# lanl-ansi/Katana.jl

Hardware: AMD Instinct MI355X
Metric: ECP iterations/sec + wall-clock to f_tol=1e-6, 1e5-var synthetic convex NLP (higher is better)
Workload: dtype f64; 1 GPU; cfg3: n=100000 variables, m_lin=50000 linear rows (8 nnz), m_nl=10000 explog rows (k=32 nnz), seed 0, planted non-degenerate vertex optimum, f_tol=1e-6; parallelism=1 GPU

## Files before the change

### katana.jl_amd/csrc/engine.hpp

```cpp
#pragma once
#include <hip/hip_runtime.h>

#include <algorithm>
#include <chrono>
#include <cstdlib>
#include <cmath>
#include <limits>
#include <map>
#include <string>
#include <vector>

#include <rccl/rccl.h>

#include "common.hpp"
#include "types.hpp"
#include "prims.hpp"

namespace ktn {

static const double kInf = std::numeric_limits<double>::infinity();

static inline int pick_group(double avg_len) {
    int g = 4;
    while (g < 64 && 2 * g <= avg_len) g <<= 1;
    return g;
}

struct LpResult {
    int status = KTN_STATUS_NONE;
    int64_t iters = 0;
    double pobj = 0.0, dobj = 0.0, row_viol = 0.0, gap = 0.0;
    double dres_rel = 0.0;
    bool exact = false;
    bool stag_exit = false;
};

struct DevParams {
    bool no_pinned_check = false, debug_load = false, no_csc_merge = false, tiled_general_build = false, debug_blocks = false,
         no_tiled_check = false, no_setup_reuse = false, debug_lp = false, no_packed = false, force_collective = false;
    int sweep_rows = 0;
    int blk_cfg = -1;
    int sweep_blocked = -1;
    int sweep_batched = -1;
    int tape_classed = -1;
    int tiled_wg = 2;
    int ecp_power = 20;
    int grp_rows = 0, grp_cols = 0;
    int tiled = -1;
    double smax_reuse = 0.0;
    int power_passes = 0;
    int omega_robust = 1;
    int packed_trips = 0;
    int first_chunk = 31;
    int stag_chunk = 0;
    int near_chunk = -1;
    int stag_checks = 2;
    double flat_factor = 0.4;
    int omega_art = 1;
    double omega_art_k = 256.0;
    double omega_art_clamp = 0.0, omega_clamp = 0.0, omega_clamp_down = 0.0;
    double ipc_timeout_s = 20.0;
    static bool flag(const char* k) { return std::getenv(k) != nullptr; }
    static int geti(const char* k, int d) { const char* v = std::getenv(k); return v ? std::atoi(v) : d; }
    static double getd(const char* k, double d) { const char* v = std::getenv(k); return v ? std::atof(v) : d; }
    void from_env() {
        no_pinned_check = flag("KTN_NO_PINNED_CHECK"); debug_load = flag("KTN_DEBUG_LOAD"); no_csc_merge = flag("KTN_NO_CSC_MERGE");
        tiled_general_build = flag("KTN_TILED_GENERAL_BUILD"); debug_blocks = flag("KTN_DEBUG_BLOCKS"); no_tiled_check = flag("KTN_NO_TILED_CHECK");
        no_setup_reuse = flag("KTN_NO_SETUP_REUSE"); debug_lp = flag("KTN_DEBUG_LP"); no_packed = flag("KTN_NO_PACKED");
        force_collective = flag("KTN_FORCE_COLLECTIVE");
        sweep_rows = geti("KTN_SWEEP_ROWS", sweep_rows); blk_cfg = geti("KTN_BLK_CFG", blk_cfg); sweep_blocked = geti("KTN_SWEEP_BLOCKED", sweep_blocked);
        sweep_batched = geti("KTN_SWEEP_BATCHED", sweep_batched); tape_classed = geti("KTN_TAPE_CLASSED", tape_classed);
        tiled_wg = geti("KTN_TILED_WG", tiled_wg); ecp_power = geti("KTN_ECP_POWER", ecp_power);
        grp_rows = geti("KTN_GRP_ROWS", grp_rows); grp_cols = geti("KTN_GRP_COLS", grp_cols); tiled = geti("KTN_TILED", tiled);
        smax_reuse = getd("KTN_SMAX_REUSE", smax_reuse); power_passes = geti("KTN_POWER_PASSES", power_passes);
        omega_robust = geti("KTN_OMEGA_ROBUST", omega_robust); packed_trips = geti("KTN_PACKED_TRIPS", packed_trips);
        first_chunk = geti("KTN_FIRST_CHUNK", first_chunk); stag_chunk = geti("KTN_STAG_CHUNK", stag_chunk); near_chunk = geti("KTN_NEAR_CHUNK", near_chunk);
        stag_checks = geti("KTN_STAG_CHECKS", stag_checks); flat_factor = getd("KTN_FLAT_FACTOR", flat_factor);
        omega_art = geti("KTN_OMEGA_ART", omega_art); omega_art_k = getd("KTN_OMEGA_ART_K", omega_art_k);
        omega_art_clamp = getd("KTN_OMEGA_ART_CLAMP", omega_art_clamp); omega_clamp = getd("KTN_OMEGA_CLAMP", omega_clamp);
        omega_clamp_down = getd("KTN_OMEGA_CLAMP_DOWN", omega_clamp_down); ipc_timeout_s = getd("KTN_IPC_TIMEOUT_S", ipc_timeout_s);
    }
};

struct Engine {
    ktn_params prm;
    DevParams dev;
    std::string err;
    hipStream_t stream = nullptr;
    int device = 0;

    bool loaded = false;
    int64_t n0 = 0, m0 = 0;
    int64_t n_lp = 0;
    int64_t m_ext = 0;
    int64_t nnz_ext = 0;
    int sense = KTN_MIN;
    bool obj_linear = true;
    bool has_inf_bound = false;
    std::vector<int64_t> h_rowptr;
    std::vector<int32_t> h_col;
    std::vector<uint8_t> h_rowkind;
    std::vector<double> h_lb, h_ub;
    std::vector<int32_t> h_nlrows;
    int64_t m_nl = 0, n_tape_nl = 0;
    int64_t m_nl_global = 0;
    int grp_sweep = 32;
    int sweep_rows_per_group = 1;
    bool pre_multirow = false;

    DBuf<int64_t> d_rowptr, d_nodeptr;
    DBuf<int32_t> d_col, d_nodeop, d_nodea, d_nodeb;
    DBuf<uint8_t> d_rowkind, d_padzero;
    DBuf<uint64_t> d_dkeys, d_dsorted;
    ktn_eval_rows_cb cb_rows = nullptr;
    ktn_eval_obj_cb cb_obj = nullptr;
    void* cb_user = nullptr;
    int64_t n_host = 0, n_host_nl = 0;
    bool host_constr_rows = false, host_obj = false;
    std::vector<double> h_xh, h_gh, h_jh;
    DBuf<double> d_gh, d_jh;
    DBuf<int32_t> d_hostrows;
    void host_eval(const double* d_x);
    DBuf<int32_t> d_colk;
    DBuf<double2> d_pp;
    bool blk_on = false;
    int blk_nb = 0, blk_cfg = 0, blk_cols = kBlkCols, blk_wg_per_cu = 2, num_cus = 256;
    DBuf<int32_t> d_bcolk;
    DBuf<double2> d_bpp;
    DBuf<int64_t> d_bseg;
    DBuf<int4> d_bkind;
    DBuf<SepSlot> d_slots;
    DBuf<SepPartial> d_part;
    DBuf<double> d_rconst, d_lb, d_ub, d_nodec, d_nodeval, d_nodeadj;
// ... 31 lines not shown
    bool lp_dirty = true;
    uint64_t lp_version = 1, scaled_version = 0, smax_version = 0;
    bool scaled_identity = false;
    ktn_exchange_cb exch_cb = nullptr;
    void* exch_user = nullptr;
    int64_t exch_lo = 0;
    bool exchanging() const { return exch_cb != nullptr; }
    bool sharded_rows = false;
    bool glists = false;
    int64_t nl_total = 0;
    int64_t last_sweep_cuts = 0;
    DBuf<int64_t> d_glast, d_nlid;
    void append_link(int64_t nrows, const int64_t* nl_id_host);
    void append_link_dev(int64_t nrows);
    int64_t* list_heads() { return glists ? d_glast.p : d_lastcut.p; }
    int64_t list_count() const { return glists ? nl_total : m_nl; }
    bool lists_ok() const { return !sharded_rows || glists; }
    DBuf<int64_t> c_ptr, c_cnt;
    DBuf<int32_t> c_row;
    DBuf<double> c_val, c_sval, r_sval;
    DBuf<uint32_t> c_perm, c_perm2;
    DBuf<int32_t> c_row2;
    DBuf<int64_t> c_ptr2, c_off;
    int64_t csc_M = -1, csc_NNZ = 0;
    uint64_t lp_epoch = 1, csc_epoch = 0;
    void csc_merge_appended();
    bool w_shift = false;
    int64_t M_lin = 0;
    DBuf<double> wval, wlo, whi, wc, epi_ref, epi_scal;
    DBuf<unsigned long long> epi_newest;
    const double* Wval() const { return w_shift ? wval.p : lp_val.p; }
    const double* Wlo() const { return w_shift ? wlo.p : lp_lo.p; }
    const double* Whi() const { return w_shift ? whi.p : lp_hi.p; }
    const double* Wc() const { return w_shift ? wc.p : lp_c.p; }
    bool want_shift(int mode) const { return prm.epi_shift != 0 && !obj_linear && mode == 0 && !row_sharded() && n_blocks == 0; }
    void build_working();
    void ensure_matrix(bool shift);
    void epi_dot(const double* x);
    DBuf<uint64_t> k_in, k_out;
    DBuf<uint32_t> p_in, p_out;
    DBuf<char> d_sorttmp;
    DBuf<double> dr_r, dc_r;
    DBuf<ColRec> d_crec;
    DBuf<RowRec> d_rrec;
    DBuf<int2> d_cbl;
    bool packed_on = false;
    int packed_trips = 1;
    DBuf<double> dr2, dc2;
    DBuf<double> dr, dc, statr, statc, ch, lh, uh, loh, hih, xh, yh, x0h, y0h, xth, yth, xbar, pv, pw, box;
    DBuf<double> partials, chk_part, chkout, power_v, power_v0;
    int64_t power_v0_n = -1;
    double* h_chk = nullptr;
    double* h_chk_dev = nullptr;
    int64_t lp_iter_budget = 0, dense_credit = 0, dense_run = 0;
    DBuf<int32_t> ds_W, ds_valid;
    DBuf<double> ds_dense, ds_out;
    DBuf<double> md_Binv, md_hW, md_x, md_lam, md_u, md_d, md_r, md_pv, md_c, md_aug, md_prow, md_fcol;
    int64_t md_since_refactor = 0;
    int64_t mid_backoff = 0, mid_backoff_len = 0;
    DBuf<int32_t> md_W, md_pi, md_lost;
    DBuf<MidState> md_st;
    bool md_valid = false;
    int64_t mid_credit = 0, mid_run = 0;
    DBuf<int32_t> d_longrows;
    DBuf<int32_t> d_longcols;
    int64_t n_longc = 0;
    int64_t col_gain_max = 0;
    int64_t col_len_max = -1, col_scan_rows = 0;
    int64_t col_removed_rows = 0;
    void find_long_cols();
    void spmv_cols(const SpMat& AT, const double* v, double* out, hipEvent_t e0 = nullptr, hipEvent_t e1 = nullptr);
    static constexpr int kMaxChunk = 512;
    int64_t n_long = 0;
    static constexpr int64_t kLongRow = 2048;
    int64_t max_row_len = (int64_t)1 << 62;
    double omega = 1.0;
    bool have_omega = false;
    int grp_rows = 8, grp_cols = 8;
    struct TiledBuf {
        DBuf<int64_t> segstart, segtot;
        DBuf<uint16_t> bptr, cur, idx;
        DBuf<int32_t> pcnt;
        DBuf<double> val;
        int nb_in = 0;
        int64_t tiles = 0, grid = 0, pieces = 1;
        TiledMat view() const { return TiledMat{segstart.p, bptr.p, idx.p, val.p, nb_in}; }
    } tA, tAT;
    DBuf<double> tpart;
    bool tiled_on = false, tiled_built = false;
    void launch_tiled(const TiledBuf& T, int64_t n_out, int64_t n_in, const double* in, hipEvent_t e0);
    bool build_tiled(TiledBuf& T, int64_t n_out, int64_t n_in, const int64_t* ptr, const int32_t* idx, const double* val, int64_t skip_longer);
    int64_t n_blocks = 0, blocks_built_rows = -1;
    size_t lds_set_lp = 0, lds_set_ecp = 0;
    std::vector<int64_t> h_blkcol;
    DBuf<int64_t> d_blkcol;
    DBuf<int32_t> d_blkrowptr, d_blkrows, d_rowloc, d_crowl;
    DBuf<double> d_blkomega, d_blkres;
    int blk_nmax = 0, blk_mmax = 0;
    void build_blocks();
    bool optimize_blocks_device(int cap_mul);
    DBuf<EcpArena> d_ar;
    DBuf<int64_t> d_blklin, d_blknl;
    DBuf<int32_t> e_rptr, e_cptr, e_last, e_prev;
    DBuf<uint16_t> e_rcol, e_crow;
    DBuf<double> e_xbest, e_ax, e_rval, e_rsval, e_lo, e_hi, e_y, e_dr, e_loh, e_hih, e_cval, e_csval, e_dc, e_ch, e_lh, e_uh, e_res;
    bool lp_solve_blocks(double tol_p, double tol_g, double eta, LpResult* R, int64_t max_it);
// ... 12 lines not shown
    int polish_count = 0;
    double polish_phi = 1e-3;
    double cert_target = 0.0;
    double cert_gap = 0.0;
    DBuf<double> d_cert;
    double objective_certificate(int64_t id_offset = 0, bool raw = false);
    double certificate_all_ranks();
    bool sweep_all(const double* d_x, double f_cut, bool lp_ok, int lp_stat, int64_t* nviol, double* maxviol, double* extra0, double* extra1);
    double certificate_blocks(double* gap_tol);
    DBuf<double> d_certblk;
    double best_viol = kInf, best_obj = 0.0;
    DBuf<double> d_xbest;
    int64_t log_cuts_lastprnt = 0, log_max_viol = 0, purged_total = 0;
    bool logging() const { return prm.log_level > 0 && dist.rank == 0; }
    void print_header() const {
        std::printf("%-10s %-15s %-15s %-20s %-20s %-15s\n", "Iteration", "Total cuts", "Cuts added", "Max constr. viol.",
                    "Avg constr. viol.", "Current cuts");
    }
    void print_stats(int64_t iter_lastprnt) const {
        const double avg = (double)log_cuts_lastprnt / ((double)iter_lastprnt * (double)m_nl);
        std::printf("%-10lld %-15lld %-15lld %-20lld %-20.2f %-15lld\n", (long long)iter, (long long)numcuts,
                    (long long)log_cuts_lastprnt, (long long)log_max_viol, avg, (long long)(numcuts - purged_total));
        std::fflush(stdout);
    }
    std::chrono::steady_clock::time_point t_start;
    std::vector<std::vector<double>> lp_sols;
    std::map<std::string, double> stats;
    std::vector<hipEvent_t> ev_pool;
    struct EvRec { int kind; size_t a, b; double bytes; };
    std::vector<EvRec> ev_recs;
    size_t ev_used = 0;

    explicit Engine(const ktn_params& p) : prm(p) {
        dev.from_env();
        if (prm.cut_algo != KTN_CUT_KELLEY && prm.cut_algo != KTN_CUT_SUPPORTING)
            throw Error(KTN_E_INVALID, "cut_algo must be KTN_CUT_KELLEY (0) or KTN_CUT_SUPPORTING (1)");
        int ndev = 0;
        if (hipGetDeviceCount(&ndev) != hipSuccess || ndev <= 0)
            throw Error(KTN_E_NODEVICE, "no HIP device visible: the Katana HIP engine has no CPU path");
        if (prm.device >= 0) {
            KTN_HIP(hipSetDevice(prm.device));
            device = prm.device;
        } else {
            KTN_HIP(hipGetDevice(&device));
        }
        {
            int cus = 0;
            if (hipDeviceGetAttribute(&cus, hipDeviceAttributeMultiprocessorCount, device) == hipSuccess && cus > 0) num_cus = cus;
        }
        KTN_HIP(hipStreamCreateWithFlags(&stream, hipStreamNonBlocking));
        partials.resize((size_t)kRedBlocks * kChkQ * 2, stream);
        chkout.resize(kChkQ * 2 + 16, stream);
        if (!dev.no_pinned_check &&
            hipHostMalloc((void**)&h_chk, sizeof(double) * (2 * kChkQ + 16), hipHostMallocMapped) == hipSuccess) {
            if (hipHostGetDevicePointer((void**)&h_chk_dev, h_chk, 0) != hipSuccess) { (void)hipHostFree(h_chk); h_chk = nullptr; h_chk_dev = nullptr; }
        } else {
            h_chk = nullptr;
            (void)hipGetLastError();
        }
        d_scal.resize(8, stream);
        d_anynf.resize(4, stream);
    }
    ~Engine() {
        delete child;
        if (dist.comm) (void)ncclCommDestroy(dist.comm);
        ipc_release();
        for (auto e : ev_pool) (void)hipEventDestroy(e);
        if (stream) (void)hipStreamDestroy(stream);
        if (h_chk) (void)hipHostFree(h_chk);
    }

    void sync() { KTN_HIP(hipStreamSynchronize(stream)); }
    bool chk_pinned() const { return h_chk_dev != nullptr && !row_sharded(); }
    double* chk_target() { return chk_pinned() ? h_chk_dev : chkout.p; }
    void check_launch() { KTN_HIP(hipGetLastError()); }

    struct DistCtx {
        int rank = 0, world = 1;
        bool force = false;
        ncclComm_t comm = nullptr;
        ktn_allreduce_cb cb = nullptr;
        void* user = nullptr;
        std::vector<double> hbuf;
        struct Ipc {
            bool on = false;
            int64_t cap = 0;
            double* data = nullptr;
            unsigned long long* flags = nullptr;
            void* opened[2 * kIpcMaxRanks] = {};
            IpcPeers P = {};
            unsigned long long epoch = 0;
            long long timeout_ticks = 0;
            int* h_err = nullptr;
            int* h_err_dev = nullptr;
        } ipc;
    } dist;
    int64_t ipc_off() const { return (int64_t)(dist.ipc.epoch & 1ull) * dist.ipc.cap; }
    double* ipc_slot() const { return dist.ipc.data + ipc_off(); }
    void ipc_check() {
        if (dist.ipc.on && dist.ipc.h_err && *dist.ipc.h_err != 0) {
            const int code = *dist.ipc.h_err;
            if (code > 100)
                throw Error(KTN_E_HIP, "peer-buffer transport: rank " + std::to_string(code - 101) + " gave up (told rank " + std::to_string(dist.rank) + ")");
            throw Error(KTN_E_HIP, "peer-buffer transport: rank " + std::to_string(dist.rank) + " timed out waiting for rank " + std::to_string(code - 1));
        }
    }
    int64_t ipc_barrier();
    void ipc_release();
    void probe_fill(int64_t n, double* v, double value);
    DBuf<double> d_red;
    bool row_sharded() const { return dist.world > 1 || dist.force; }
    void allreduce(double* d, size_t n, int op);
    void allreduce_host(double* v, int k, int op);

    size_t ev_get() {
        if (ev_used == ev_pool.size()) {
            hipEvent_t e;
            KTN_HIP(hipEventCreate(&e));
            ev_pool.push_back(e);
        }
// ... 48 lines not shown
    DBuf<double2> d_sbpp;
    DBuf<int64_t> d_sbseg;

    std::vector<int8_t> h_esh_side;
    DBuf<int8_t> d_esh_sig;
    DBuf<double> d_xint, d_lam;
    DBuf<int32_t> d_tape_nlslots;
    DBuf<unsigned long long> d_esh_cnt;
    std::vector<double> h_xint;
    bool xint_given = false, esh_ready = false;
    int xint_found = 0;
    int64_t esh_n_part = 0;
    struct EshAux {
        int64_t n = 0, m = 0;
        std::vector<double> lv, uv, lc, uc, rconst, p0, p1, targ, op0, op1;
        std::vector<int64_t> rowptr, tptr;
        std::vector<int32_t> col, top, ocol;
        std::vector<uint8_t> kind, lin, akind, okind;
        bool has_tape = false;
    } aux;
    Engine* child = nullptr;
    void esh_build_aux(const double* l_var, const double* u_var, const double* l_constr, const double* u_constr, const ktn_nlp_desc* d);
    void esh_prepare();
    void esh_find_interior();
    bool esh_on = false;
    int64_t esh_last_rows = 0;
    void esh_search(const double* d_x, double f_tol);
    void esh_emit(const double* d_x, int64_t V);
    DBuf<int32_t> d_esh_one;
    DBuf<int64_t> d_esh_slot;
    bool esh_gencut_row(int64_t i, double* coefs, double* constant);
    void esh_last_lambdas(double* out);

    void rebuild_csc();
    void purge_cuts();
    void reserve_lp(int64_t rows, int64_t nnz);
    void find_long_rows();
    bool recession_ray_dense(bool* unbounded);
    void launch_y(const SpMat& A, double sigma, double w, double rho, hipEvent_t e0, hipEvent_t e1);
    void launch_x(const SpMat& AT, double tau, double w, double rho, bool update, hipEvent_t e0, hipEvent_t e1);
    bool launch_check(const SpMat& A, const SpMat& AT, double tau, double sigma, double w_next = -1.0, double rho = 1.0);
    DBuf<double> xnext, ynext;
    int chk_nrow = 0, chk_ncol = 0;
    void compute_scaling(bool identity);
    LpResult lp_solve(double tol_p, double tol_g, int mode, bool identity_scaling = false);
    LpResult lp_solve_core(double tol_p, double tol_g, int mode, bool identity_scaling);
    bool lp_solve_dense(LpResult* R);
    bool lp_solve_mid(LpResult* R);
    void pdhg_raw(const double* x0, const double* y0, double eta, double omega_, int64_t iters, double* x_out,
                  double* y_out);
    void lp_pick_groups();
    void lp_choose_tiled(bool same_matrix);
    void lp_set_anchors(bool want_packed);
    void lp_read_check(double* q);
    void lp_restart();
    void lp_advance(bool spec, int64_t k, double rho);
    struct LpScriptIO {
        const double *x, *y, *x0, *y0;
        double eta, omega;
        int64_t k;
        int32_t flags;
        const int32_t* ops;
        int64_t nops;
        double *x_out, *y_out, *x0_out, *y0_out, *xt_out, *yt_out, *q_out, *xnext_out, *ynext_out;
        int32_t* spec_out;
        double *dr_out, *dc_out;
    };
    void lp_script(const LpScriptIO& io);
    void lp_scaling(double* dr_out, double* dc_out, double* drr_out, double* dcr_out);

    bool recession_ray();
    void boundroutine();
    void begin();
    void step(int32_t* done);
    void polish_step(int32_t* done);
    void end();
};

}
```

### katana.jl_amd/csrc/lp.hip

```cpp
#include "engine.hpp"
#include "launch.hpp"
#include "kernels.hpp"
#include "dense_lp.hpp"
#include "mid_lp.hpp"
#include "batch_lp.hpp"

namespace ktn {

double Engine::dev_dot(int64_t n, const double* a, const double* b) {
    hipLaunchKernelGGL(k_dot_partial, dim3(kRedBlocks), dim3(kBlock), 0, stream, n, a, b, partials.p);
    hipLaunchKernelGGL(k_sum_final, dim3(1), dim3(kRedBlocks), 0, stream, partials.p, kRedBlocks, chkout.p + 2 * kChkQ);
    double v = 0.0;
    KTN_HIP(hipMemcpyAsync(&v, chkout.p + 2 * kChkQ, sizeof(double), hipMemcpyDeviceToHost, stream));
    sync();
    return v;
}

double Engine::dev_finite_sq(int64_t n, const double* a) {
    hipLaunchKernelGGL(k_finite_sq_partial, dim3(kRedBlocks), dim3(kBlock), 0, stream, n, a, partials.p);
    hipLaunchKernelGGL(k_sum_final, dim3(1), dim3(kRedBlocks), 0, stream, partials.p, kRedBlocks, chkout.p + 2 * kChkQ);
    double v = 0.0;
    KTN_HIP(hipMemcpyAsync(&v, chkout.p + 2 * kChkQ, sizeof(double), hipMemcpyDeviceToHost, stream));
    sync();
    return v;
// ... 601 lines not shown
        md_valid = false;
        ok = true;
    }
    stats["lp_time_s"] += std::chrono::duration<double>(std::chrono::steady_clock::now() - t0).count();
    return ok;
}

void Engine::lp_pick_groups() {
    const int64_t n = n_lp, m = M;
    const double avg_r = m ? (double)NNZ / (double)m : 1.0, avg_c = n ? (double)NNZ / (double)n : 1.0;
    grp_rows = pick_group(avg_r);
    grp_cols = pick_group(avg_c);
    if (dev.grp_rows > 0) grp_rows = dev.grp_rows;
    if (dev.grp_cols > 0) grp_cols = dev.grp_cols;
}

void Engine::lp_choose_tiled(bool same_matrix) {
    {
        const bool tenv = dev.tiled >= 0;
        const int64_t units_t = ceil_div(M, (int64_t)kTileOut) * ceil_div(n_lp, (int64_t)kTileIn);
        const int64_t units_tt = ceil_div(n_lp, (int64_t)kTileOut) * ceil_div(M, (int64_t)kTileIn);
        tiled_on = prm.lp_tiled_nnz > 0 && NNZ >= prm.lp_tiled_nnz && n_lp >= 2 * kTileIn && M >= 2 * kTileIn &&
                   NNZ >= 4096 * std::max(units_t, units_tt);
        if (tenv) tiled_on = dev.tiled != 0 && M > 0 && NNZ > 0;
        if (same_matrix) tiled_on = tiled_built;
        else if (tiled_on) {
            auto tt = std::chrono::steady_clock::now();
            tiled_on = build_tiled(tA, M, n_lp, lp_rowptr.p, lp_col.p, r_sval.p, kLongRow) &&
                       build_tiled(tAT, n_lp, M, c_ptr.p, c_row.p, c_sval.p, (int64_t)1 << 62);
            tpart.resize((size_t)std::max<int64_t>(tA.pieces * M, tAT.pieces * n_lp), stream);
            stats["lp_tiled_builds"] += 1.0;
            stats["lp_tiled_build_time_s"] += std::chrono::duration<double>(std::chrono::steady_clock::now() - tt).count();
            if (!tiled_on) stats["lp_tiled_overflows"] += 1.0;
        }
        tiled_built = tiled_on;
    }
}

void Engine::lp_set_anchors(bool want_packed) {
    const int64_t n = n_lp, m = M;
    const size_t mm = (size_t)std::max<int64_t>(m, 1);
    packed_on = want_packed && !tiled_on && !row_sharded() && NNZ < ((int64_t)1 << 31) && !dev.no_packed;
    if (dev.packed_trips > 0) packed_trips = dev.packed_trips;
    if (packed_on) {
        d_crec.resize((size_t)n, stream); d_cbl.resize((size_t)n, stream); d_rrec.resize(mm, stream);
        LAUNCH_1(k_pack_both, std::max(n, m), stream, n, c_ptr.p, ch.p, lh.p, uh.p, xh.p, x0h.p, d_crec.p, d_cbl.p,
                 m, lp_rowptr.p, loh.p, hih.p, yh.p, y0h.p, d_rrec.p);
    } else {
        KTN_HIP(hipMemcpyAsync(x0h.p, xh.p, n * sizeof(double), hipMemcpyDeviceToDevice, stream));
        if (m > 0) KTN_HIP(hipMemcpyAsync(y0h.p, yh.p, m * sizeof(double), hipMemcpyDeviceToDevice, stream));
    }
}

void Engine::lp_read_check(double* q) {
    if (chk_pinned()) {
        sync();
        std::memcpy(q, h_chk, 2 * kChkQ * sizeof(double));
    } else {
        KTN_HIP(hipMemcpyAsync(q, chkout.p, 2 * kChkQ * sizeof(double), hipMemcpyDeviceToHost, stream));
        sync();
        ipc_check();
    }
}

void Engine::lp_restart() {
    const int64_t n = n_lp, m = M;
    LAUNCH_1(k_restart_set, std::max(n, m), stream, n, m, xth.p, xh.p, x0h.p, yth.p, yh.p, y0h.p, packed_on ? d_crec.p : (ColRec*)nullptr,
             packed_on ? d_rrec.p : (RowRec*)nullptr);
}

void Engine::lp_advance(bool spec, int64_t k, double rho) {
    const int64_t n = n_lp, m = M;
    if (spec) {
        xh.swap(xnext); yh.swap(ynext);
    } else {
        const double w = (double)(k + 1) / (double)(k + 2);
        LAUNCH_1(k_halpern2, std::max(n, m), stream, n, m, xh.p, xth.p, x0h.p, yh.p, yth.p, y0h.p, w, rho);
    }
}

LpResult Engine::lp_solve_core(double tol_p, double tol_g, int mode, bool identity_scaling) {
    auto t0 = std::chrono::steady_clock::now();
    LpResult R;
    auto lap = [&](const char* key, std::chrono::steady_clock::time_point& tp) {
        if (!prm.profile) return;
        sync();
        const auto now = std::chrono::steady_clock::now();
        stats[key] += std::chrono::duration<double>(now - tp).count();
        tp = now;
    };
    auto tp = t0;
    ensure_matrix(want_shift(mode));
    lap("lp_csc_time_s", tp);
    const bool no_reuse = dev.no_setup_reuse;
    const bool same_matrix = !no_reuse && !row_sharded() && scaled_version == lp_version && scaled_identity == identity_scaling;
    find_long_rows();
    if (!same_matrix) compute_scaling(identity_scaling);
    else stats["lp_setup_reuses"] += 1.0;
    lap("lp_scaling_time_s", tp);
    const int64_t n = n_lp, m = M;
    const size_t mm = (size_t)std::max<int64_t>(m, 1);
    ch.resize(n, stream); lh.resize(n, stream); uh.resize(n, stream); xh.resize(n, stream);
    x0h.resize(n, stream); xth.resize(n, stream); xbar.resize(n, stream); pv.resize(n, stream);
    loh.resize(mm, stream); hih.resize(mm, stream); yh.resize(mm, stream); y0h.resize(mm, stream);
    yth.resize(mm, stream); pw.resize(mm, stream);
    const double sgn = (sense == KTN_MAX) ? -1.0 : 1.0;
    LAUNCH_1(k_prep_both, std::max(n, m), stream,
             PrepCols{n, Wc(), lp_l.p, lp_u.p, dc.p, lp_x.p, (mode == 1 ? box.p : (const double*)nullptr), sgn, mode, ch.p, lh.p, uh.p, xh.p},
             PrepRows{m, Wlo(), Whi(), dr.p, lp_y.p, mode, loh.p, hih.p, yh.p});
    if (w_shift) {
        epi_dot(lp_x.p);
        hipLaunchKernelGGL(k_epi_var, dim3(1), dim3(1), 0, stream, xh.p, (int32_t)n0, epi_scal.p, (const double*)dc.p, -1, have_omega ? 0 : 1, sgn, epi_newest.p);
    }
    check_launch();
    lp_pick_groups();
    SpMat A{lp_rowptr.p, lp_col.p, r_sval.p};
    SpMat AT{c_ptr.p, c_row.p, c_sval.p};
    lp_choose_tiled(same_matrix);
    scaled_version = lp_version; scaled_identity = identity_scaling;

    double smax = 0.0;
    bool have_power = false;
    const double smax_reuse = dev.smax_reuse;
    const bool reuse_smax = mode == 0 && smax_reuse > 0.0 && smax_rows > 0 && m >= smax_rows && !row_sharded() &&
                            (double)(m - smax_rows) <= smax_reuse * (double)smax_rows && smax_prev > 0.0;
    if (same_matrix && smax_version == lp_version && smax_prev > 0.0) smax = smax_prev;
    else if (reuse_smax) { smax = smax_prev; stats["lp_smax_reused"] += 1.0; }
    else if ((m > 0 && NNZ > 0) || row_sharded()) {
        double* nrm = (chk_pinned() ? h_chk_dev : chkout.p) + 2 * kChkQ + 1;
        auto dot_dev = [&](const double* a, double* out) {
            hipLaunchKernelGGL(k_dot_partial, dim3(kRedBlocks), dim3(kBlock), 0, stream, n, a, a, partials.p);
            hipLaunchKernelGGL(k_sum_final, dim3(1), dim3(kRedBlocks), 0, stream, partials.p, kRedBlocks, out);
        };
        auto normalize_into = [&](const double* a, double* out) {
            hipLaunchKernelGGL(k_dot_partial, dim3(kRedBlocks), dim3(kBlock), 0, stream, n, a, a, partials.p);
            hipLaunchKernelGGL(k_normalize_sum, dim3(ceil_div(n, (int64_t)kRedBlocks)), dim3(kRedBlocks), 0, stream, n, a, partials.p, out);
        };
        if (power_v0_n != n) {
            power_v.resize(n, stream); power_v0.resize(n, stream);
            LAUNCH_1(k_hash_fill, n, stream, n, power_v.p);
            normalize_into(power_v.p, power_v0.p);
            power_v0_n = n;
        }
        const int passes_env = dev.power_passes;
        const int iters = passes_env > 0 ? passes_env : 8;
        for (int it = 0; it < iters; ++it) {
            const double* vin = (it == 0) ? power_v0.p : pv.p;
            if (n_long > 0) {
                LAUNCH_G(grp_rows, k_spmv_skip, m, stream, m, A, vin, pw.p, kLongRow);
// ... 44 lines not shown
        const double nv2 = hs[1];
        smax = (nv2 > 0.0) ? std::sqrt(std::sqrt(nv2)) : 0.0;
        if (mode == 0) { smax_prev = smax; smax_rows = m; smax_version = lp_version; }
    }
    lap("lp_power_time_s", tp);
    double fro2 = (NNZ > 0) ? hs[2] : 0.0;
    allreduce_host(&fro2, 1, 0);
    const double fro = std::sqrt(fro2);
    if (!(smax > 0.0)) smax = fro;
    const double eta_safe = 0.998 / std::max(identity_scaling ? fro : std::min(1.0, fro), 1e-12);
    double eta = std::max(0.998 / std::max(smax, 1e-12), eta_safe);
    int stall = 0, grow = 0, flat_rows = 0, consolidations = 0, infeas_hits = 0;
    double pobj_h[3] = {1e300, -1e300, 1e300}, pviol_h[3] = {1e300, -1e300, 1e300};
    double r_last_check = 0.0;
    stats["lp_setup_time_s"] += std::chrono::duration<double>(std::chrono::steady_clock::now() - t0).count();
    const double nc2 = hs[3];
    const double nc2_tol = w_shift ? hs[6] : nc2;
    double nb2 = (m > 0) ? hs[4] + hs[5] : 0.0;
    allreduce_host(&nb2, 1, 0);
    double omega_ref = (nc2 > 0.0 && nb2 > 0.0) ? std::sqrt(nc2 / nb2) : 1.0;
    if (robust && hs[9] > 0.0 && hs[11] > 0.0) {
        omega_ref = std::sqrt(hs[9] / hs[11]) * std::exp(hs[8] / hs[9] - hs[10] / hs[11]);
        stats["lp_omega_robust"] += 1.0;
    }
    double om = (have_omega && mode == 0) ? omega : omega_ref;
    const double rho = 1.0;
    const double cinf_scale = 1.0;
    if (dev.debug_lp)
        std::fprintf(stderr, "[lp setup mode %d] m %lld n %lld nnz %lld smax %.4g fro %.4g nc2 %.4g nc2_tol %.4g nb2 %.4g omega_ref %.4g om0 %.4g shift %d b_ref %.9g n_long %lld tol_p %.3g tol_g %.3g\n",
                     mode, (long long)m, (long long)n, (long long)NNZ, smax, fro, nc2, nc2_tol, nb2, omega_ref, om, (int)w_shift, epi_b, (long long)n_long, tol_p, tol_g);

    lp_set_anchors(true);

    const double ky_bytes = (double)NNZ * 12 + 8.0 * (m + 1) + 8.0 * 5 * m + 8.0 * n;
    const double kx_bytes = (double)NNZ * 12 + 8.0 * (n + 1) + 8.0 * 7 * n + 8.0 * m;
    int64_t k = 0, it = 0;
    double r0 = 0.0, r_prev = 0.0;
    const bool dbg_lp = dev.debug_lp;
    R.status = KTN_STATUS_USERLIMIT;
    const int64_t max_it = lp_iter_budget > 0 ? std::min<int64_t>(lp_iter_budget, prm.lp_max_iter) : prm.lp_max_iter;
    const int chk = std::max(1, prm.lp_check_every);
    const int plain_len = std::min(chk - 1, (int)kMaxChunk);
    const int first_chunk = dev.first_chunk;
    bool plain_next = false, near_conv = false, primal_ok = false;
    const int stag_chunk = dev.stag_chunk;
    bool blocks_done = false;
    if (n_blocks > 0 && mode == 0 && !row_sharded() && n_long == 0 && m > 0 && !prm.profile) {
        if (blocks_built_rows != M) build_blocks();
        blocks_done = lp_solve_blocks(tol_p, tol_g, eta, &R, max_it);
        if (blocks_done) it = R.iters;
    }
    const int near_env = dev.near_chunk;
    const int near_chunk = near_env >= 0 ? near_env : prm.lp_near_check;
    while (!blocks_done && it < max_it) {
        const double tau = eta / om, sigma = eta * om;
        if (plain_next) {
            plain_next = false;
            int want = (k <= 1 && first_chunk > 0) ? std::min(first_chunk, plain_len) : plain_len;
            if (near_conv && near_chunk > 0) want = std::min(want, near_chunk);
            if (primal_ok && stag_chunk > 0 && mode == 0) want = std::min(want, stag_chunk);
            const int np = (int)std::min<int64_t>(want, max_it - it);
            if (np <= 0) continue;
            for (int j = 0; j < np; ++j) {
                const double w = (double)(k + j + 1) / (double)(k + j + 2);
                if (prm.profile) {
                    const size_t e0 = ev_get(), e1 = ev_get(), e2 = ev_get(), e3 = ev_get();
                    launch_x(AT, tau, w, rho, true, ev_pool[e0], ev_pool[e1]);
                    launch_y(A, sigma, w, rho, ev_pool[e2], ev_pool[e3]);
                    ev_recs.push_back({0, e0, e1, kx_bytes});
                    if (m > 0) ev_recs.push_back({1, e2, e3, ky_bytes});
                } else {
                    launch_x(AT, tau, w, rho, true, nullptr, nullptr);
                    launch_y(A, sigma, w, rho, nullptr, nullptr);
                }
            }
            k += np; it += np;
            continue;
        }
        const bool spec_next = launch_check(A, AT, tau, sigma, (double)(k + 1) / (double)(k + 2), rho);
        check_launch();
        double q[2 * kChkQ];
        lp_read_check(q);
        if (prm.profile) ev_flush();
        const double dyAdx = q[0], dy2 = q[1], dobj_rows = q[2], dy0sq = q[3], yt2 = q[4], pviol = q[12];
        const double dx2 = q[kChkQ + 5], pobj = q[kChkQ + 6] + obj_shift, dobj_cols = q[kChkQ + 7], dx0sq = q[kChkQ + 8],
                     xt2 = q[kChkQ + 9], dres = q[kChkQ + 13];
        const double dobj = dobj_rows + dobj_cols + obj_shift;
        const double r2 = om / eta * dx2 - 2.0 * dyAdx + dy2 / (eta * om);
        const double r = std::sqrt(std::max(r2, 0.0));
        const double gap = std::fabs(pobj - dobj) / (1.0 + std::fabs(pobj) + std::fabs(dobj));
        if (k == 0) { r0 = r; r_prev = r; }
        if (dbg_lp) std::fprintf(stderr, "[lp mode %d] it %7lld k %6lld r %.3e pviol %.3e dres %.3e gap %.3e pobj %.10g dobj %.10g om %.3g eta %.3g\n",
                                 mode, (long long)it, (long long)k, r, pviol, dres, gap, pobj, dobj, om, eta);
        R.pobj = pobj; R.dobj = dobj; R.row_viol = pviol; R.gap = gap;
        R.dres_rel = dres * cinf_scale / (1.0 + std::sqrt(nc2_tol));
        bool done = (pviol <= tol_p) && (gap <= tol_g) && (dres * cinf_scale <= tol_g * (1.0 + std::sqrt(nc2_tol)));
        near_conv = (pviol <= 4.0 * tol_p) && (gap <= 4.0 * tol_g) && (dres * cinf_scale <= 4.0 * tol_g * (1.0 + std::sqrt(nc2_tol)));
        primal_ok = (pviol <= tol_p) && (dres * cinf_scale <= tol_g * (1.0 + std::sqrt(nc2_tol)));
        {
            const bool boxed_free = has_inf_bound;
            const double stag = boxed_free ? std::min(prm.lp_stag_factor, 100.0) : prm.lp_stag_factor;
            if (stag > 0.0 && mode == 0 && !done) {
                const double scale = 1.0 + std::fabs(pobj);
                const int stag_checks = dev.stag_checks;
                const double flat_f = dev.flat_factor;
                const double ff = boxed_free ? std::min(flat_f, 0.1) : flat_f;
                const int nchk = boxed_free ? 3 : stag_checks;
                const bool flat = std::fabs(pobj - pobj_h[0]) <= ff * tol_g * scale && std::fabs(pobj - pobj_h[1]) <= ff * tol_g * scale &&
                                  (nchk < 3 || std::fabs(pobj - pobj_h[2]) <= ff * tol_g * scale);
                const double accept0 = (tol_p > prm.lp_tol_floor * prm.f_tol * (1.0 + 1e-9)) ? 10.0 : 3.0;
                const bool plateau = pviol <= accept0 * tol_p && std::fabs(pviol - pviol_h[0]) <= 0.02 * pviol &&
                                     std::fabs(pviol - pviol_h[1]) <= 0.02 * pviol && std::fabs(pviol - pviol_h[2]) <= 0.02 * pviol;
                if (flat && (pviol <= tol_p || plateau) && gap <= stag * tol_g && dres * cinf_scale <= tol_g * (1.0 + std::sqrt(nc2_tol))) {
                    done = true;
                    R.stag_exit = true;
                    stats["lp_stagnation_exits"] += 1.0;
                }
            }
            const double stall_accept = (tol_p > prm.lp_tol_floor * prm.f_tol * (1.0 + 1e-9)) ? 10.0 : 3.0;
            if (stag > 0.0 && mode == 0 && !done && gap <= tol_g && dres * cinf_scale <= tol_g * (1.0 + std::sqrt(nc2_tol)) &&
                pviol <= stall_accept * tol_p && std::fabs(pviol - pviol_h[0]) <= 0.02 * pviol && std::fabs(pviol - pviol_h[1]) <= 0.02 * pviol &&
                std::fabs(pviol - pviol_h[2]) <= 0.02 * pviol) {
                done = true;
                stats["lp_stalled_row_exits"] += 1.0;
            }
            pviol_h[2] = pviol_h[1]; pviol_h[1] = pviol_h[0]; pviol_h[0] = pviol;
            pobj_h[2] = pobj_h[1]; pobj_h[1] = pobj_h[0]; pobj_h[0] = pobj;
        }
        if (done || !(r == r)) {
            R.status = done ? KTN_STATUS_OPTIMAL : KTN_STATUS_ERROR;
            ++it;
            break;
        }
        if (mode == 0 && (m > 0 || row_sharded())) {
            const double farkas = dobj_rows + q[kChkQ + 10];
// ... 16 lines not shown
                if (grow >= 2) stats["lp_divergence_backoffs"] += 1.0;
                stall = 0; grow = 0;
                restart = true;
                stats["lp_eta_backoffs"] += 1.0;
            }
        }
        const bool have_lists = row_sharded() ? (prm.lp_dual_inherit != 0) : (prm.lp_dual_inherit && lists_ok() && list_count() > 0 && m > M_base);
        if (mode == 0 && k > 0 && have_lists && gap <= tol_g &&
            dres * cinf_scale <= tol_g * (1.0 + std::sqrt(nc2_tol)) && pviol > tol_p) {
            flat_rows = (r_last_check > 0.0 && r > 0.98 * r_last_check) ? flat_rows + 1 : 0;
            if (flat_rows >= 3 && consolidations < 8) {
                flat_rows = 0;
                ++consolidations;
                stats["lp_consolidations"] += 1.0;
                LAUNCH_1(k_unscale, n, stream, n, xth.p, dc.p, pv.p);
                SpMat Au{lp_rowptr.p, lp_col.p, Wval()};
                LAUNCH_G(grp_rows, k_spmv, m, stream, m, Au, pv.p, pw.p);
                KTN_HIP(hipMemsetAsync(d_anynf.p + 1, 0, sizeof(int32_t), stream));
                LAUNCH_1(k_consolidate, list_count(), stream, list_count(), list_heads(), d_cutprev.p, pw.p, Wlo(), Whi(), dr.p, tol_p, yth.p,
                         d_anynf.p + 1);
                lp_restart();
                k = 0;
                r_last_check = 0.0;
                ++it;
                continue;
            }
        } else {
            flat_rows = 0;
        }
        r_last_check = r;
        r_prev = r;
        if (restart) {
            const double dx = std::sqrt(dx0sq), dy = std::sqrt(dy0sq);
            if (dbg_lp) std::fprintf(stderr, "[lp restart] it %lld k %lld decayed %d dx %.3e dy %.3e |xt| %.3e |yt| %.3e om %.4g\n", (long long)it, (long long)k, (int)decayed, dx, dy, std::sqrt(xt2), std::sqrt(yt2), om);
            const int om_art = dev.omega_art;
            const double om_art_k = dev.omega_art_k, om_art_clamp = dev.omega_art_clamp;
            if ((om_art || decayed) && dx > 1e-8 * (1.0 + std::sqrt(xt2)) && dy > 1e-8 * (1.0 + std::sqrt(yt2))) {
                const double om_clamp = dev.omega_clamp;
                const double om_old = om;
                const double theta = (!decayed && om_art_k > 0.0 && !has_inf_bound) ? 0.5 * std::min(1.0, (double)k / om_art_k) : 0.5;
                om = std::exp(theta * std::log(dy / dx) + (1.0 - theta) * std::log(om));
                if (!decayed && om_art_clamp > 1.0) om = std::min(std::max(om, om_old / om_art_clamp), om_old * om_art_clamp);
                const double om_clamp_dn = dev.omega_clamp_down;
                if (om_clamp > 1.0) om = std::min(std::max(om, om_old / om_clamp), om_old * om_clamp);
                if (om_clamp_dn > 1.0) om = std::max(om, om_old / om_clamp_dn);
                om = std::min(std::max(om, omega_ref * 1e-3), omega_ref * 1e3);
            }
            lp_restart();
            stats["lp_restarts"] += 1.0;
            k = 0;
            ++it;
            continue;
        }
        lp_advance(spec_next, k, rho);
        ++k; ++it;
        plain_next = true;
    }
    R.iters = it;
    if (mode == 0) {
        LAUNCH_1(k_unscale2, std::max(n, m), stream, n, xth.p, dc.p, lp_x.p, m, yth.p, dr.p, lp_y.p);
        if (w_shift) {
            epi_dot(lp_x.p);
            hipLaunchKernelGGL(k_epi_var, dim3(1), dim3(1), 0, stream, lp_x.p, (int32_t)n0, epi_scal.p, (const double*)nullptr, 1, 0, sgn, epi_newest.p);
        }
        omega = om;
        have_omega = true;
        objval = sgn * R.pobj + c0;
    } else {
        LAUNCH_1(k_unscale, n, stream, n, xth.p, dc.p, d_ray.p);
    }
    check_launch();
    sync();
    if (prm.profile) ev_flush();
    stats["pdhg_iters"] += (double)it;
    stats["lp_solves"] += 1.0;
    stats["lp_last_row_viol"] = R.row_viol; stats["lp_last_gap"] = R.gap; stats["lp_last_dres_rel"] = R.dres_rel;
    stats["lp_last_stag_exit"] = R.stag_exit ? 1.0 : 0.0;
    stats["lp_time_s"] += std::chrono::duration<double>(std::chrono::steady_clock::now() - t0).count();
    return R;
}

void Engine::pdhg_raw(const double* x0, const double* y0, double eta, double omega_, int64_t iters, double* x_out,
                      double* y_out) {
    ensure_matrix(false);
    compute_scaling(true);
    scaled_version = 0;
    const int64_t n = n_lp, m = M;
    const size_t mm = (size_t)std::max<int64_t>(m, 1);
    ch.resize(n, stream); lh.resize(n, stream); uh.resize(n, stream); xh.resize(n, stream);
    x0h.resize(n, stream); xth.resize(n, stream); xbar.resize(n, stream); pv.resize(n, stream);
    loh.resize(mm, stream); hih.resize(mm, stream); yh.resize(mm, stream); y0h.resize(mm, stream); yth.resize(mm, stream); pw.resize(mm, stream);
    const double sgn = (sense == KTN_MAX) ? -1.0 : 1.0;
    KTN_HIP(hipMemcpyAsync(lp_x.p, x0, n * sizeof(double), hipMemcpyHostToDevice, stream));
    if (m > 0) KTN_HIP(hipMemcpyAsync(lp_y.p, y0, m * sizeof(double), hipMemcpyHostToDevice, stream));
    LAUNCH_1(k_prep_cols, n, stream, n, lp_c.p, lp_l.p, lp_u.p, dc.p, lp_x.p, (double*)nullptr, sgn, 0, ch.p, lh.p, uh.p, xh.p);
    LAUNCH_1(k_prep_rows, m, stream, m, lp_lo.p, lp_hi.p, dr.p, lp_y.p, 0, loh.p, hih.p, yh.p);
    grp_rows = pick_group(m ? (double)NNZ / (double)m : 1.0);
    grp_cols = pick_group(n ? (double)NNZ / (double)n : 1.0);
    SpMat A{lp_rowptr.p, lp_col.p, r_sval.p};
    SpMat AT{c_ptr.p, c_row.p, c_sval.p};
    packed_on = false;
    KTN_HIP(hipMemcpyAsync(x0h.p, xh.p, n * sizeof(double), hipMemcpyDeviceToDevice, stream));
    if (m > 0) KTN_HIP(hipMemcpyAsync(y0h.p, yh.p, m * sizeof(double), hipMemcpyDeviceToDevice, stream));
    find_long_rows();
    {
        const bool tenv = dev.tiled >= 0;
        const int64_t units_t = ceil_div(M, (int64_t)kTileOut) * ceil_div(n_lp, (int64_t)kTileIn);
        const int64_t units_tt = ceil_div(n_lp, (int64_t)kTileOut) * ceil_div(M, (int64_t)kTileIn);
        tiled_on = prm.lp_tiled_nnz > 0 && NNZ >= prm.lp_tiled_nnz && n_lp >= 2 * kTileIn && M >= 2 * kTileIn &&
                   NNZ >= 4096 * std::max(units_t, units_tt);
        if (tenv) tiled_on = dev.tiled != 0 && M > 0 && NNZ > 0;
        if (tiled_on) {
            auto tt = std::chrono::steady_clock::now();
            tiled_on = build_tiled(tA, M, n_lp, lp_rowptr.p, lp_col.p, r_sval.p, kLongRow) &&
                       build_tiled(tAT, n_lp, M, c_ptr.p, c_row.p, c_sval.p, (int64_t)1 << 62);
            tpart.resize((size_t)std::max<int64_t>(tA.pieces * M, tAT.pieces * n_lp), stream);
            stats["lp_tiled_builds"] += 1.0;
            stats["lp_tiled_build_time_s"] += std::chrono::duration<double>(std::chrono::steady_clock::now() - tt).count();
            if (!tiled_on) stats["lp_tiled_overflows"] += 1.0;
        }
    }
    const double tau = eta / omega_, sigma = eta * omega_;
    const double ky_bytes = (double)NNZ * 12 + 8.0 * (m + 1) + 8.0 * 5 * m + 8.0 * n;
    const double kx_bytes = (double)NNZ * 12 + 8.0 * (n + 1) + 8.0 * 7 * n + 8.0 * m;
    for (int64_t k = 0; k < iters; ++k) {
// ... 172 lines not shown
```

### katana.jl_amd/csrc/sweep.hip

```cpp
#include <cstring>
#include <unordered_map>

#include "engine.hpp"
#include "launch.hpp"
#include "kernels.hpp"
#include "tape_classes.hpp"
#include "batch_lp.hpp"
#include "batch_ecp.hpp"

namespace ktn {

static void postfix_to_nodes(const int32_t* op, const double* arg, int64_t len, const int32_t* rcols, int64_t rlen,
                             int64_t jac_base, std::vector<int64_t>& slot_of, std::vector<int32_t>& nop,
                             std::vector<int32_t>& na, std::vector<int32_t>& nb, std::vector<double>& nc) {
    std::vector<int32_t> st;
    const int64_t base = (int64_t)nop.size();
    for (int64_t s = rlen - 1; s >= 0; --s) slot_of[(size_t)rcols[s]] = s;
    struct Reset {
        std::vector<int64_t>& m; const int32_t* c; int64_t n;
        ~Reset() { for (int64_t s = 0; s < n; ++s) m[(size_t)c[s]] = -1; }
    } reset{slot_of, rcols, rlen};
    for (int64_t t = 0; t < len; ++t) {
        const int o = op[t];
        int32_t a = 0, b = 0;
// ... 895 lines not shown
    *maxviol_out = mv;
    int64_t cap = (prm.cut_cap_factor > 0.0) ? std::max<int64_t>((int64_t)(prm.cut_cap_factor * (double)n_lp), prm.cut_cap_min) : 0;
    if (cap > 0 && row_sharded()) cap = std::max<int64_t>(cap / dist.world, 1);
    if (cap > 0 && V > cap && !anynf) {
        d_dkeys.resize((size_t)m_nl, stream); d_dsorted.resize((size_t)m_nl, stream);
        LAUNCH_1(k_depth_keys, m_nl, stream, P, d_nlrows.p, m_nl, d_g.p, d_flag.p, d_dkeys.p);
        const size_t need = sort_keys_desc_temp_bytes((size_t)m_nl);
        d_sorttmp.resize(need + 16, stream);
        KTN_HIP(sort_keys_desc_u64(d_sorttmp.p, need, d_dkeys.p, d_dsorted.p, (size_t)m_nl, stream));
        LAUNCH_1(k_depth_reflag, m_nl, stream, m_nl, d_dkeys.p, d_dsorted.p, cap, d_flag.p, d_cnt.p);
        check_launch();
        exclusive_scan(d_flag.p, d_rank.p, (size_t)m_nl);
        exclusive_scan(d_cnt.p, d_cntscan.p, (size_t)m_nl);
        KTN_HIP(hipMemcpyAsync(&tail[0], d_flag.p + (m_nl - 1), 8, hipMemcpyDeviceToHost, stream));
        KTN_HIP(hipMemcpyAsync(&tail[1], d_rank.p + (m_nl - 1), 8, hipMemcpyDeviceToHost, stream));
        KTN_HIP(hipMemcpyAsync(&tail[2], d_cnt.p + (m_nl - 1), 8, hipMemcpyDeviceToHost, stream));
        KTN_HIP(hipMemcpyAsync(&tail[3], d_cntscan.p + (m_nl - 1), 8, hipMemcpyDeviceToHost, stream));
        sync();
        V = tail[0] + tail[1];
        nnzV = tail[2] + tail[3];
        stats["cut_selections"] += 1.0;
        stats["cuts_skipped"] += (double)(*nviol_out - V);
    }
    if (anynf) {
        std::fprintf(stderr, "WARNING: Nonlinear constraint or objective likely undefined within domain\n");
        *nonfinite_out = true;
        return;
    }
    if (V > 0) {
        if (prm.cut_algo == KTN_CUT_SUPPORTING) esh_search(d_x, f_tol);
        lp_rowptr.resize((size_t)(M + V + 1), stream);
        lp_lo.resize((size_t)(M + V), stream);
        lp_hi.resize((size_t)(M + V), stream);
        lp_y.resize((size_t)(M + V), stream);
        d_cutprev.resize((size_t)(M + V), stream);
        d_age.resize((size_t)(M + V), stream);
        KTN_HIP(hipMemsetAsync(d_age.p + M, 0, (size_t)V * sizeof(int32_t), stream));
        lp_col.resize((size_t)(NNZ + nnzV), stream);
        lp_val.resize((size_t)(NNZ + nnzV), stream);
        d_violslots.resize((size_t)V, stream);
        LpRows L = lp_view();
        LAUNCH_1(k_compact, m_nl, stream, P, d_nlrows.p, m_nl, d_flag.p, d_rank.p, d_cntscan.p, d_bconst.p, M, NNZ, L,
                 d_violslots.p, d_lastcut.p, d_cutprev.p, (int)(prm.lp_dual_inherit && !glists));
        if (prm.cut_algo == KTN_CUT_SUPPORTING) esh_emit(d_x, V);
        else LAUNCH_G(grp_sweep, k_emit, V, stream, P, d_nlrows.p, d_violslots.p, V, d_x, d_jac.p, d_maxc.p,
                      prm.cut_coef_rng, 1, M, L);
        check_launch();
        M += V;
        NNZ += nnzV;
        numcuts += V;
        last_sweep_cuts = V;
        lp_dirty = true; ++lp_version;
    }
    sync();
    stats["sep_time_s"] += std::chrono::duration<double>(std::chrono::steady_clock::now() - t0).count();
}

void Engine::global_sweep(const double* d_x, double f_tol, int64_t* nviol, double* maxviol, bool* nonfinite) {
    sweep(d_x, f_tol, nviol, maxviol, nonfinite);
    if (!row_sharded()) return;
    double v[2] = {(double)*nviol, *nonfinite ? 1.0 : 0.0};
    allreduce_host(v, 2, 0);
    double mv = *maxviol;
    allreduce_host(&mv, 1, 1);
    *nviol = (int64_t)(v[0] + 0.5);
    *nonfinite = v[1] > 0.0;
    *maxviol = mv;
}

}
```

Baseline: 348.2 ECP iterations/s.

## Speculatively queue PDHG iterations behind convergence checks and drop redundant stream syncs

After launching a convergence check, the solver records an event, swaps in the speculative next iterate and enqueues up to a few further PDHG x/y iterations before the host reads the check result. The host waits on the event rather than the whole stream, so the GPU keeps running while the host decides. Queued iterations are counted toward the next chunk or discarded when the check ends the solve. It also makes the pinned check buffer coherent and skips the end-of-LP and end-of-sweep stream syncs in single-device, non-profiled mode. The trade-off is extra work when speculation is wasted, and correctness now depends on later stream ordering instead of explicit drains.

```diff
diff --git a/katana.jl_amd/csrc/engine.hpp b/katana.jl_amd/csrc/engine.hpp
--- a/katana.jl_amd/csrc/engine.hpp
+++ b/katana.jl_amd/csrc/engine.hpp
@@ -60,6 +60,7 @@
     double omega_art_k = 256.0;
     double omega_art_clamp = 0.0, omega_clamp = 0.0, omega_clamp_down = 0.0;
     double ipc_timeout_s = 20.0;
+    int spec_iters = -1;
     static bool flag(const char* k) { return std::getenv(k) != nullptr; }
     static int geti(const char* k, int d) { const char* v = std::getenv(k); return v ? std::atoi(v) : d; }
     static double getd(const char* k, double d) { const char* v = std::getenv(k); return v ? std::atof(v) : d; }
@@ -79,6 +80,7 @@
         omega_art = geti("KTN_OMEGA_ART", omega_art); omega_art_k = getd("KTN_OMEGA_ART_K", omega_art_k);
         omega_art_clamp = getd("KTN_OMEGA_ART_CLAMP", omega_art_clamp); omega_clamp = getd("KTN_OMEGA_CLAMP", omega_clamp);
         omega_clamp_down = getd("KTN_OMEGA_CLAMP_DOWN", omega_clamp_down); ipc_timeout_s = getd("KTN_IPC_TIMEOUT_S", ipc_timeout_s);
+        spec_iters = std::min(geti("KTN_SPEC_ITERS", spec_iters), 8);
     }
 };
 
@@ -216,6 +218,12 @@
     int64_t power_v0_n = -1;
     double* h_chk = nullptr;
     double* h_chk_dev = nullptr;
+    static constexpr int kSpecIters = 3;
+    hipEvent_t spec_ev = nullptr;
+    int spec_depth() const { return dev.spec_iters < 0 ? kSpecIters : dev.spec_iters; }
+    bool drains_dropped() const {
+        return dev.spec_iters != 0 && !prm.profile && !row_sharded() && !exchanging() && cb_rows == nullptr && cb_obj == nullptr;
+    }
     int64_t lp_iter_budget = 0, dense_credit = 0, dense_run = 0;
     DBuf<int32_t> ds_W, ds_valid;
     DBuf<double> ds_dense, ds_out;
@@ -334,8 +342,9 @@
         partials.resize((size_t)kRedBlocks * kChkQ * 2, stream);
         chkout.resize(kChkQ * 2 + 16, stream);
         if (!dev.no_pinned_check &&
-            hipHostMalloc((void**)&h_chk, sizeof(double) * (2 * kChkQ + 16), hipHostMallocMapped) == hipSuccess) {
+            hipHostMalloc((void**)&h_chk, sizeof(double) * (2 * kChkQ + 16), hipHostMallocMapped | hipHostMallocCoherent) == hipSuccess) {
             if (hipHostGetDevicePointer((void**)&h_chk_dev, h_chk, 0) != hipSuccess) { (void)hipHostFree(h_chk); h_chk = nullptr; h_chk_dev = nullptr; }
+            else if (hipEventCreateWithFlags(&spec_ev, hipEventDisableTiming) != hipSuccess) { spec_ev = nullptr; (void)hipGetLastError(); }
         } else {
             h_chk = nullptr;
             (void)hipGetLastError();
@@ -348,6 +357,7 @@
         if (dist.comm) (void)ncclCommDestroy(dist.comm);
         ipc_release();
         for (auto e : ev_pool) (void)hipEventDestroy(e);
+        if (spec_ev) (void)hipEventDestroy(spec_ev);
         if (stream) (void)hipStreamDestroy(stream);
         if (h_chk) (void)hipHostFree(h_chk);
     }
@@ -502,7 +512,7 @@
     void lp_pick_groups();
     void lp_choose_tiled(bool same_matrix);
     void lp_set_anchors(bool want_packed);
-    void lp_read_check(double* q);
+    void lp_read_check(double* q, bool by_event = false);
     void lp_restart();
     void lp_advance(bool spec, int64_t k, double rho);
     struct LpScriptIO {
diff --git a/katana.jl_amd/csrc/lp.hip b/katana.jl_amd/csrc/lp.hip
--- a/katana.jl_amd/csrc/lp.hip
+++ b/katana.jl_amd/csrc/lp.hip
@@ -677,9 +677,10 @@
     }
 }
 
-void Engine::lp_read_check(double* q) {
+void Engine::lp_read_check(double* q, bool by_event) {
     if (chk_pinned()) {
-        sync();
+        if (by_event) KTN_HIP(hipEventSynchronize(spec_ev));
+        else sync();
         std::memcpy(q, h_chk, 2 * kChkQ * sizeof(double));
     } else {
         KTN_HIP(hipMemcpyAsync(q, chkout.p, 2 * kChkQ * sizeof(double), hipMemcpyDeviceToHost, stream));
@@ -720,6 +721,7 @@
     const bool no_reuse = dev.no_setup_reuse;
     const bool same_matrix = !no_reuse && !row_sharded() && scaled_version == lp_version && scaled_identity == identity_scaling;
     find_long_rows();
+    if (n_long > 0) stats["lp_long_row_solves"] += 1.0;
     if (!same_matrix) compute_scaling(identity_scaling);
     else stats["lp_setup_reuses"] += 1.0;
     lap("lp_scaling_time_s", tp);
@@ -870,8 +872,13 @@
     }
     const int near_env = dev.near_chunk;
     const int near_chunk = near_env >= 0 ? near_env : prm.lp_near_check;
+    const int spec_S = spec_depth();
+    const bool spec_ok = spec_S > 0 && packed_on && !prm.profile && chk_pinned() && spec_ev != nullptr;
+    int spec_queued = 0;
+    int spec_unused = 0;
     while (!blocks_done && it < max_it) {
         const double tau = eta / om, sigma = eta * om;
+        if (spec_unused > 0) { stats["lp_spec_discarded"] += (double)spec_unused; spec_unused = 0; }
         if (plain_next) {
             plain_next = false;
             int want = (k <= 1 && first_chunk > 0) ? std::min(first_chunk, plain_len) : plain_len;
@@ -879,7 +886,10 @@
             if (primal_ok && stag_chunk > 0 && mode == 0) want = std::min(want, stag_chunk);
             const int np = (int)std::min<int64_t>(want, max_it - it);
             if (np <= 0) continue;
-            for (int j = 0; j < np; ++j) {
+            KTN_REQUIRE(spec_queued <= np, "lp_solve_core: speculation outran the chunk");
+            const int j0 = spec_queued;
+            spec_queued = 0;
+            for (int j = j0; j < np; ++j) {
                 const double w = (double)(k + j + 1) / (double)(k + j + 2);
                 if (prm.profile) {
                     const size_t e0 = ev_get(), e1 = ev_get(), e2 = ev_get(), e3 = ev_get();
@@ -897,8 +907,27 @@
         }
         const bool spec_next = launch_check(A, AT, tau, sigma, (double)(k + 1) / (double)(k + 2), rho);
         check_launch();
+        bool spec_swapped = false;
+        if (spec_ok && spec_next && it + 1 < max_it) {
+            KTN_HIP(hipEventRecord(spec_ev, stream));
+            xh.swap(xnext); yh.swap(ynext);
+            spec_swapped = true;
+            int64_t cand = std::min<int64_t>(plain_len, max_it - it - 1);
+            if (k == 0 && first_chunk > 0) cand = std::min<int64_t>(cand, first_chunk);
+            if (near_chunk > 0) cand = std::min<int64_t>(cand, near_chunk);
+            if (stag_chunk > 0 && mode == 0) cand = std::min<int64_t>(cand, stag_chunk);
+            const int sq = (int)std::max<int64_t>(std::min<int64_t>(spec_S, cand), 0);
+            for (int j = 0; j < sq; ++j) {
+                const double w = (double)(k + 1 + j + 1) / (double)(k + 1 + j + 2);
+                launch_x(AT, tau, w, rho, true, nullptr, nullptr);
+                launch_y(A, sigma, w, rho, nullptr, nullptr);
+            }
+            check_launch();
+            spec_unused = sq;
+            stats["lp_spec_launched"] += (double)sq;
+        }
         double q[2 * kChkQ];
-        lp_read_check(q);
+        lp_read_check(q, spec_swapped);
         if (prm.profile) ev_flush();
         const double dyAdx = q[0], dy2 = q[1], dobj_rows = q[2], dy0sq = q[3], yt2 = q[4], pviol = q[12];
         const double dx2 = q[kChkQ + 5], pobj = q[kChkQ + 6] + obj_shift, dobj_cols = q[kChkQ + 7], dx0sq = q[kChkQ + 8],
@@ -1021,10 +1050,12 @@
             ++it;
             continue;
         }
-        lp_advance(spec_next, k, rho);
+        if (!spec_swapped) lp_advance(spec_next, k, rho);
+        spec_queued = spec_unused; spec_unused = 0;
         ++k; ++it;
         plain_next = true;
     }
+    if (spec_unused > 0) { stats["lp_spec_discarded"] += (double)spec_unused; spec_unused = 0; }
     R.iters = it;
     if (mode == 0) {
         LAUNCH_1(k_unscale2, std::max(n, m), stream, n, xth.p, dc.p, lp_x.p, m, yth.p, dr.p, lp_y.p);
@@ -1039,7 +1070,7 @@
         LAUNCH_1(k_unscale, n, stream, n, xth.p, dc.p, d_ray.p);
     }
     check_launch();
-    sync();
+    if (mode != 0 || !drains_dropped()) sync();
     if (prm.profile) ev_flush();
     stats["pdhg_iters"] += (double)it;
     stats["lp_solves"] += 1.0;
diff --git a/katana.jl_amd/csrc/sweep.hip b/katana.jl_amd/csrc/sweep.hip
--- a/katana.jl_amd/csrc/sweep.hip
+++ b/katana.jl_amd/csrc/sweep.hip
@@ -971,7 +971,7 @@
         last_sweep_cuts = V;
         lp_dirty = true; ++lp_version;
     }
-    sync();
+    if (!drains_dropped()) sync();
     stats["sep_time_s"] += std::chrono::duration<double>(std::chrono::steady_clock::now() - t0).count();
 }
 
```

Result: no change. 346.3 ECP iterations/s (-0.6%).
